# memgraph/memgraph

Hardware: AMD Instinct MI355X
Metric: edges/s PageRank (higher is better)
Workload: dtype f32; 1 GPU; RMAT-26 PageRank (327 iters); scale=26, vertices=67108864, edges=1073741824, seed=1, accumulation=f64-per-row, parallelism=single

## Files before the change

include/mgx_analytics.h:

```cpp
#ifndef MGX_ANALYTICS_H
#define MGX_ANALYTICS_H

#include <stddef.h>
#include <stdint.h>

#ifdef __cplusplus
extern "C" {
#endif

typedef int32_t mgx_status;
#define MGX_OK 0
#define MGX_ERR_NO_DEVICE 1
#define MGX_ERR_HIP 2
#define MGX_ERR_INVALID_ARGUMENT 3
#define MGX_ERR_TOO_LARGE 4
#define MGX_ERR_OUT_OF_MEMORY 5
#define MGX_ERR_NCCL 6
#define MGX_ERR_NOT_SUPPORTED 7

const char *mgx_status_string(mgx_status s);
const char *mgx_last_error(void);

int mgx_device_count(void);

typedef struct mgx_context mgx_context;
typedef struct mgx_graph mgx_graph;

mgx_status mgx_init(int device, mgx_context **out);
mgx_status mgx_destroy(mgx_context *ctx);
mgx_status mgx_sync(mgx_context *ctx);


#define MGX_BUILD_IN_CSR 1u
#define MGX_BUILD_SYM_CSR 2u
#define MGX_BUILD_WEIGHTED 4u
#define MGX_BUILD_OUT_CSR 8u
#define MGX_BUILD_NO_PERM 16u

mgx_status mgx_graph_from_coo(mgx_context *ctx, const int64_t *src, const int64_t *dst,
                              const double *weights, int64_t n_vertices, int64_t n_edges,
                              uint32_t flags, mgx_graph **out);

mgx_status mgx_graph_rmat(mgx_context *ctx, int scale, int64_t n_edges, uint64_t seed,
                          double a, double b, double c, uint32_t flags, uint64_t weight_seed,
                          mgx_graph **out);
mgx_status mgx_graph_uniform(mgx_context *ctx, int64_t n_vertices, int64_t n_edges,
                             uint64_t seed, uint32_t flags, uint64_t weight_seed,
                             mgx_graph **out);

mgx_status mgx_graph_rmat_sharded(mgx_context *ctx, int scale, int64_t n_edges, uint64_t seed,
                                  double a, double b, double c, int64_t row_begin,
                                  int64_t row_end, mgx_graph **out);

mgx_status mgx_gen_edges_to_host(mgx_context *ctx, int rmat, int scale, int64_t n_vertices,
                                 int64_t n_edges, uint64_t seed, double a, double b,
                                 double c, int64_t *out_src, int64_t *out_dst);

mgx_status mgx_graph_destroy(mgx_context *ctx, mgx_graph *g);
int64_t mgx_graph_num_vertices(const mgx_graph *g);
int64_t mgx_graph_num_edges(const mgx_graph *g);
int64_t mgx_graph_local_edges(const mgx_graph *g);
double mgx_graph_build_ms(const mgx_graph *g);
int64_t mgx_graph_in_zero_rows(const mgx_graph *g);
int64_t mgx_graph_xcd_heavy_rows(const mgx_graph *g);


typedef struct {
  int64_t iterations;
  double iter_ms;
  double sweep_ms;
  int64_t sweep_launches;
  double csr_build_ms;
  double download_ms;
} mgx_pagerank_stats;

mgx_status mgx_pagerank(mgx_context *ctx, mgx_graph *g, int64_t max_iterations,
                        double damping_factor, double stop_epsilon, double *out_rank,
                        mgx_pagerank_stats *stats);

typedef struct mgx_pagerank_run mgx_pagerank_run;
mgx_status mgx_pagerank_start(mgx_context *ctx, mgx_graph *g, double damping_factor,
                              mgx_pagerank_run **out);
mgx_status mgx_pagerank_iterate(mgx_pagerank_run *run, int64_t n_iterations);
mgx_status mgx_pagerank_iterate_eps(mgx_pagerank_run *run, int64_t max_n,
                                    double stop_epsilon, int64_t *done);
int64_t mgx_pagerank_xcd_lds_floats(const mgx_pagerank_run *run);
int mgx_pagerank_xcd_block_threads(const mgx_pagerank_run *run);
mgx_status mgx_pagerank_timing(mgx_pagerank_run *run, double *sweep_ms, int64_t *launches);
mgx_status mgx_pagerank_finish(mgx_pagerank_run *run, double *out_rank );

mgx_status mgx_wcc(mgx_context *ctx, mgx_graph *g, int64_t *out_component,
                   int64_t *n_components);

#define MGX_BFS_AUTO 0
#define MGX_BFS_TOP_DOWN 1
#define MGX_BFS_BOTTOM_UP 2
typedef struct {
  int64_t depth;
  int64_t reached;
  int64_t entries_scanned;
  int64_t top_down_levels, bottom_up_levels;
  uint64_t bottom_up_mask;
  double ms;
} mgx_bfs_stats;
mgx_status mgx_bfs(mgx_context *ctx, mgx_graph *g, int64_t source, int directed,
                   int64_t max_depth , int mode,
                   int64_t *out_hops , int64_t *out_parent ,
                   mgx_bfs_stats *stats );

typedef struct {
  int64_t bridges, trees, depth;
  int64_t nontree_entries;
  int64_t level_launches;
  double forest_ms, ms;
} mgx_bridges_stats;
mgx_status mgx_bridges(mgx_context *ctx, mgx_graph *g, int64_t *out_u, int64_t *out_v,
                       int64_t *n_bridges, mgx_bridges_stats *stats );
// ... 94 lines not shown
```

memgraph_amd/csrc/graph_build.hip:

```cpp

#include <cstring>

#include <rocprim/rocprim.hpp>

#include "../../include/mgx_graphgen.h"
#include "mgx_device.h"
#include "mgx_xcd_deal.h"

namespace {

__global__ void k_rmat(int64_t n_edges, int scale, uint64_t mixed_seed,
                       mgx_rmat_thresholds t, int32_t *src, int32_t *dst) {
  for (int64_t i = blockIdx.x * (int64_t)blockDim.x + threadIdx.x; i < n_edges;
       i += (int64_t)gridDim.x * blockDim.x) {
    uint64_t s, d;
    mgx_rmat_edge(mixed_seed, (uint64_t)i, scale, t, &s, &d);
    src[i] = (int32_t)s;
    dst[i] = (int32_t)d;
  }
}

__global__ void k_uniform(int64_t n_edges, uint64_t mixed_seed, uint64_t n_vertices,
                          int32_t *src, int32_t *dst) {
  for (int64_t i = blockIdx.x * (int64_t)blockDim.x + threadIdx.x; i < n_edges;
       i += (int64_t)gridDim.x * blockDim.x) {
    uint64_t s, d;
    mgx_uniform_edge(mixed_seed, (uint64_t)i, n_vertices, &s, &d);
    src[i] = (int32_t)s;
    dst[i] = (int32_t)d;
  }
}

__global__ void k_weights(int64_t n_edges, uint64_t mixed_seed, float *w) {
  for (int64_t i = blockIdx.x * (int64_t)blockDim.x + threadIdx.x; i < n_edges;
       i += (int64_t)gridDim.x * blockDim.x) {
    w[i] = (float)mgx_edge_weight(mixed_seed, (uint64_t)i);
  }
}

__global__ void k_hist(int64_t n_edges, const int32_t *idx, uint32_t *counts) {
  for (int64_t i = blockIdx.x * (int64_t)blockDim.x + threadIdx.x; i < n_edges;
       i += (int64_t)gridDim.x * blockDim.x)
    atomicAdd(&counts[idx[i]], 1u);
}

__global__ void k_hist2(int64_t n_edges, const int32_t *a, const int32_t *b,
                        uint32_t *counts) {
  for (int64_t i = blockIdx.x * (int64_t)blockDim.x + threadIdx.x; i < n_edges;
       i += (int64_t)gridDim.x * blockDim.x) {
    atomicAdd(&counts[a[i]], 1u);
    atomicAdd(&counts[b[i]], 1u);
  }
}

__global__ void k_hist_ranged(int64_t n_edges, const int32_t *idx, int32_t lo, int32_t hi,
                              uint32_t *counts ) {
  for (int64_t i = blockIdx.x * (int64_t)blockDim.x + threadIdx.x; i < n_edges;
       i += (int64_t)gridDim.x * blockDim.x) {
    int32_t v = idx[i];
    if (v >= lo && v < hi) atomicAdd(&counts[v - lo], 1u);
// ... 287 lines not shown
mgx_status mgx_build_bins(mgx_context *ctx, const uint32_t *row_ptr, int64_t rows,
                          mgx_bins *bins) {
  return mgx_build_bins_range(ctx, row_ptr, row_ptr + 1, rows, true,
                              bins);
}

namespace {
__global__ void k_stripe_search(int64_t rows, const uint32_t *row_ptr, const int32_t *col,
                                int32_t boundary, uint32_t *out) {
  for (int64_t r = blockIdx.x * (int64_t)blockDim.x + threadIdx.x; r < rows;
       r += (int64_t)gridDim.x * blockDim.x) {
    uint32_t lo = row_ptr[r], hi = row_ptr[r + 1];
    while (lo < hi) {
      uint32_t mid = (lo + hi) / 2;
      if (col[mid] < boundary) lo = mid + 1;
      else hi = mid;
    }
    out[r] = lo;
  }
}

__global__ void k_xcd_search(int64_t nH, const int32_t *H, const uint32_t *row_ptr,
                             const int32_t *col, int64_t V, uint32_t *out) {
  for (int64_t s = blockIdx.x * (int64_t)blockDim.x + threadIdx.x; s < nH;
       s += (int64_t)gridDim.x * blockDim.x) {
    const int32_t r = H[s];
    const uint32_t end = row_ptr[r + 1];
    uint32_t lo = row_ptr[r];
    out[s] = lo;
    for (int x = 1; x < kXcdStripes; ++x) {
      const int32_t boundary = (int32_t)mgx_xcd_stripe_off(V, x);
      uint32_t hi = end;
      while (lo < hi) {
        const uint32_t mid = lo + (hi - lo) / 2;
        if (col[mid] < boundary) lo = mid + 1;
        else hi = mid;
      }
      out[(size_t)x * nH + s] = lo;
    }
    out[(size_t)kXcdStripes * nH + s] = end;
  }
}

__global__ void k_xcd_deal(int64_t n, const int32_t *order_sorted, const uint32_t *deg_sorted,
                           int32_t *order, uint32_t *deg) {
  for (int64_t p = blockIdx.x * (int64_t)blockDim.x + threadIdx.x; p < n;
       p += (int64_t)gridDim.x * blockDim.x) {
    const int64_t id = mgx_xcd_deal(p, n);
    order[id] = order_sorted[p];
    deg[id] = deg_sorted[p];
  }
}

mgx_status build_xcd_view(mgx_context *ctx, mgx_graph *g) {
  int heavy_min = 64;
  if (const char *e = getenv("MGX_PR_XCD_HEAVY_MIN")) {
    const int v = atoi(e);
    if (v == 8 || v == 64 || v == 1024) heavy_min = v;
  }
  const int sec = heavy_min == 8 ? 1 : heavy_min == 64 ? 2 : 3;
  g->xcd_heavy_min = heavy_min;
  g->xcd_heavy_sec = sec;
  int64_t light = 0, nH = 0;
  for (int b = 0; b < 4; ++b) (b < sec ? light : nH) += g->bins_in.count[b];
  g->xcd_nH = nH;
  if (nH == 0) return MGX_OK;
  g->xcd_H = g->bins_in.rows + light;
  MGX_HIP_TRY(mgx_hip_malloc(&g->xcd_ptr, (size_t)(kXcdStripes + 1) * nH * sizeof(uint32_t)));
  hipLaunchKernelGGL(k_xcd_search, dim3(grid_for(nH)), dim3(kBlock), 0, ctx->stream, nH,
                     g->xcd_H, g->in_row_ptr, g->in_col, g->n_vertices, g->xcd_ptr);
  for (int x = 0; x < kXcdStripes; ++x) {
    MGX_TRY(mgx_build_bins_range(ctx, g->xcd_ptr + (size_t)x * nH,
                                 g->xcd_ptr + (size_t)(x + 1) * nH, nH,
                                 false, &g->xcd_bins[x]));
  }
  mgx_bin_sections secs[kXcdStripes];
  for (int x = 0; x < kXcdStripes; ++x) (void)mgx_fill_sections(g->xcd_bins[x], &secs[x]);
  MGX_HIP_TRY(mgx_hip_malloc(&g->xcd_sec, sizeof(secs)));
  MGX_HIP_TRY(hipMemcpyAsync(g->xcd_sec, secs, sizeof(secs), hipMemcpyHostToDevice,
                             ctx->stream));
  MGX_HIP_TRY(hipStreamSynchronize(ctx->stream));
  return MGX_OK;
}
}

bool mgx_xcd_wanted(int64_t n_vertices) {
  const char *stripes = getenv("MGX_PR_STRIPES");
  if (stripes && atoi(stripes) > 0) return false;
  const char *e = getenv("MGX_PR_XCD");
  if (e && *e) return atoi(e) != 0;
  return n_vertices >= (int64_t)3 << 24;
}

mgx_status mgx_build_stripes(mgx_context *ctx, mgx_graph *g) {
  const int64_t rows = g->row_end - g->row_begin;
  const int64_t V = g->n_vertices;
  if (g->xcd) {
    g->n_stripes = 1;
    return build_xcd_view(ctx, g);
  }
  int n_stripes = 1;
  const char *env = getenv("MGX_PR_STRIPES");
  if (env && atoi(env) > 0) {
    n_stripes = atoi(env);
  } else if (g->order == nullptr) {
    const int64_t contrib_bytes = V * 4;
    n_stripes = (int)((contrib_bytes + (96 << 20) - 1) / (96 << 20));
    if (n_stripes < 1) n_stripes = 1;
  } else {
    n_stripes = 1;
  }
  if (n_stripes > 16) n_stripes = 16;
  g->n_stripes = n_stripes;
  if (n_stripes == 1) return MGX_OK;
  g->stripe_width = (V + n_stripes - 1) / n_stripes;

  MGX_HIP_TRY(mgx_hip_malloc(&g->stripe_ptr, (size_t)(n_stripes + 1) * rows * sizeof(uint32_t)));
  struct CopyK {
    static __global__ void shift(int64_t rows, const uint32_t *row_ptr, uint32_t *lo,
                                 uint32_t *hi) {
      for (int64_t r = blockIdx.x * (int64_t)blockDim.x + threadIdx.x; r < rows;
           r += (int64_t)gridDim.x * blockDim.x) {
        lo[r] = row_ptr[r];
        hi[r] = row_ptr[r + 1];
      }
    }
  };
  hipLaunchKernelGGL(CopyK::shift, dim3(grid_for(rows)), dim3(kBlock), 0, ctx->stream, rows,
                     g->in_row_ptr, g->stripe_ptr, g->stripe_ptr + (size_t)n_stripes * rows);
  for (int sIdx = 1; sIdx < n_stripes; ++sIdx) {
    hipLaunchKernelGGL(k_stripe_search, dim3(grid_for(rows)), dim3(kBlock), 0, ctx->stream,
                       rows, g->in_row_ptr, g->in_col,
                       (int32_t)((int64_t)sIdx * g->stripe_width),
                       g->stripe_ptr + (size_t)sIdx * rows);
  }
// ... 261 lines not shown
```

memgraph_amd/csrc/mgx_api.cpp:

```cpp

#include <atomic>
#include <cstdarg>
#include <cstdio>
#include <cstring>

#include "mgx_internal.h"

namespace {
thread_local char g_error[1024] = {0};
}

void mgx_set_error(const char *fmt, ...) {
  va_list ap;
  va_start(ap, fmt);
  vsnprintf(g_error, sizeof(g_error), fmt, ap);
  va_end(ap);
}

extern "C" const char *mgx_last_error(void) { return g_error; }

extern "C" const char *mgx_status_string(mgx_status s) {
  switch (s) {
    case MGX_OK: return "ok";
    case MGX_ERR_NO_DEVICE: return "no HIP device";
// ... 328 lines not shown
  if (row_begin < 0 || row_end < row_begin) {
    mgx_set_error("bad shard range [%lld,%lld)", (long long)row_begin, (long long)row_end);
    return MGX_ERR_INVALID_ARGUMENT;
  }
  MGX_HIP_TRY(hipSetDevice(ctx->device));
  mgx_graph *g = nullptr;
  mgx_status s;
  {
    mgx_scope coo(ctx);
    int32_t *d_src = nullptr, *d_dst = nullptr;
    MGX_TRY(coo.alloc_plain(&d_src, n_edges));
    MGX_TRY(coo.alloc_plain(&d_dst, n_edges));
    s = mgx_gen_rmat_device(ctx, scale, n_edges, seed, a, b, c, d_src, d_dst);
    if (s == MGX_OK) {
      g = new mgx_graph();
      const int64_t clamped_end = row_end < V ? row_end : V;
      s = mgx_build_sharded_in_csr(ctx, d_src, d_dst, V, n_edges, row_begin, clamped_end, g);
      if (s == MGX_OK) {
        g->row_end = row_end;
      }
    }
  }
  if (s != MGX_OK) {
    if (g) (void)mgx_graph_destroy(ctx, g);
    return s;
  }
  *out = g;
  return MGX_OK;
}

extern "C" mgx_status mgx_graph_destroy(mgx_context *ctx, mgx_graph *g) {
  if (!g) return MGX_OK;
  (void)ctx;
  if (g->in_row_ptr) (void)hipFree(g->in_row_ptr);
  if (g->in_col) (void)hipFree(g->in_col);
  if (g->out_degree) (void)hipFree(g->out_degree);
  if (g->inv_outdeg) (void)hipFree(g->inv_outdeg);
  if (g->out_row_ptr) (void)hipFree(g->out_row_ptr);
  if (g->out_col) (void)hipFree(g->out_col);
  if (g->in_w) (void)hipFree(g->in_w);
  if (g->bins_out.rows) (void)hipFree(g->bins_out.rows);
  if (g->sym_row_ptr) (void)hipFree(g->sym_row_ptr);
  if (g->sym_col) (void)hipFree(g->sym_col);
  if (g->sym_w) (void)hipFree(g->sym_w);
  if (g->bins_in.rows) (void)hipFree(g->bins_in.rows);
  if (g->bins_sym.rows) (void)hipFree(g->bins_sym.rows);
  if (g->stripe_ptr) (void)hipFree(g->stripe_ptr);
  if (g->order) (void)hipFree(g->order);
  for (int i = 0; i < 16; ++i) {
    if (g->stripe_bins[i].rows) (void)hipFree(g->stripe_bins[i].rows);
  }
  if (g->xcd_ptr) (void)hipFree(g->xcd_ptr);
  if (g->xcd_sec) (void)hipFree(g->xcd_sec);
  for (int i = 0; i < 8; ++i) {
    if (g->xcd_bins[i].rows) (void)hipFree(g->xcd_bins[i].rows);
  }
  if (!g->uniq_alias) {
    if (g->uniq_row_ptr) (void)hipFree(g->uniq_row_ptr);
    if (g->uniq_col) (void)hipFree(g->uniq_col);
  }
  if (g->uniq_bins.rows) (void)hipFree(g->uniq_bins.rows);
  delete g;
  return MGX_OK;
}

extern "C" int64_t mgx_graph_num_vertices(const mgx_graph *g) { return g->n_vertices; }
extern "C" int64_t mgx_graph_num_edges(const mgx_graph *g) { return g->n_edges; }
extern "C" int64_t mgx_graph_local_edges(const mgx_graph *g) { return g->in_edges; }
extern "C" double mgx_graph_build_ms(const mgx_graph *g) { return g->build_ms; }
extern "C" int64_t mgx_graph_in_zero_rows(const mgx_graph *g) { return g->bins_in.n_zero; }
extern "C" int64_t mgx_graph_xcd_heavy_rows(const mgx_graph *g) {
  return g->xcd ? g->xcd_nH : -1;
}

extern "C" mgx_status mgx_wcc(mgx_context *ctx, mgx_graph *g, int64_t *out_component,
                              int64_t *n_components) {
  MGX_HIP_TRY(hipSetDevice(ctx->device));
  return mgx_wcc_impl(ctx, g, out_component, n_components);
}

extern "C" mgx_status mgx_bfs(mgx_context *ctx, mgx_graph *g, int64_t source, int directed,
                              int64_t max_depth, int mode, int64_t *out_hops,
                              int64_t *out_parent, mgx_bfs_stats *stats) {
  MGX_HIP_TRY(hipSetDevice(ctx->device));
  return mgx_bfs_impl(ctx, g, source, directed, max_depth, mode, out_hops, out_parent, stats);
}

extern "C" mgx_status mgx_bridges(mgx_context *ctx, mgx_graph *g, int64_t *out_u,
                                  int64_t *out_v, int64_t *n_bridges,
                                  mgx_bridges_stats *stats) {
  MGX_HIP_TRY(hipSetDevice(ctx->device));
  return mgx_bridges_impl(ctx, g, out_u, out_v, n_bridges, stats);
}

extern "C" mgx_status mgx_bridges_state(mgx_context *ctx, mgx_graph *g, int64_t *parent,
                                        int64_t *level, int64_t *pre, int64_t *nd,
                                        int64_t *low, int64_t *high) {
  MGX_HIP_TRY(hipSetDevice(ctx->device));
  return mgx_bridges_state_impl(ctx, g, parent, level, pre, nd, low, high);
}

extern "C" void mgx_bridges_last_stage_ms(double *forest, double *sorts_scans, double *sweep,
                                          double *levels) {
  mgx_bridges_last_stage_ms_impl(forest, sorts_scans, sweep, levels);
}

extern "C" mgx_status mgx_similarity_pairs(mgx_context *ctx, mgx_graph *g, int metric,
                                           int mode, const int64_t *u, const int64_t *v,
                                           int64_t n_pairs, double *out_sim,
                                           int64_t *out_common, mgx_similarity_stats *stats) {
  MGX_HIP_TRY(hipSetDevice(ctx->device));
  return mgx_similarity_pairs_impl(ctx, g, metric, mode, u, v, n_pairs, out_sim, out_common,
                                   stats);
}

extern "C" mgx_status mgx_similarity_all(mgx_context *ctx, mgx_graph *g, int metric,
                                         double *out_sim, mgx_similarity_stats *stats) {
  MGX_HIP_TRY(hipSetDevice(ctx->device));
  return mgx_similarity_all_impl(ctx, g, metric, out_sim, stats);
}

extern "C" mgx_status mgx_katz(mgx_context *ctx, mgx_graph *g, double alpha, double epsilon,
                               double *out_centrality, int64_t *iterations) {
  MGX_HIP_TRY(hipSetDevice(ctx->device));
  return mgx_katz_impl(ctx, g, alpha, epsilon, out_centrality, iterations);
}
// ... 13 lines not shown
```

memgraph_amd/csrc/mgx_internal.h:

```cpp
#ifndef MGX_INTERNAL_H
#define MGX_INTERNAL_H

#include <hip/hip_runtime.h>

#include <cstdint>
#include <cstdio>
#include <map>
#include <mutex>
#include <string>
#include <unordered_map>
#include <vector>

#include "../../include/mgx_analytics.h"

void mgx_set_error(const char *fmt, ...);

#define MGX_HIP_TRY(expr)                                                     \
  do {                                                                        \
    hipError_t _e = (expr);                                                   \
    if (_e != hipSuccess) {                                                   \
      mgx_set_error("%s:%d: %s failed: %s", __FILE__, __LINE__, #expr,        \
                    hipGetErrorString(_e));                                   \
      (void)hipGetLastError();  \
      return MGX_ERR_HIP;                                                     \
// ... 74 lines not shown
  int64_t count[4] = {0, 0, 0, 0};
  int64_t n_zero = 0;
  int64_t grid[4] = {0, 0, 0, 0};
  int64_t total_grid() const { return grid[0] + grid[1] + grid[2] + grid[3]; }
};

inline int64_t mgx_bin_grid(int b, int64_t count) {
  const int64_t rows_per_block[4] = {64, 16, 4, 1};
  const int64_t cap[4] = {2048, 2048, 2048, 8192};
  const int64_t need = (count + rows_per_block[b] - 1) / rows_per_block[b];
  return count ? (need < cap[b] ? need : cap[b]) : 0;
}

struct mgx_graph {
  int64_t n_vertices = 0;
  int64_t n_edges = 0;
  uint32_t flags = 0;

  uint32_t *in_row_ptr = nullptr;
  int32_t *in_col = nullptr;
  int64_t in_edges = 0;
  int64_t row_begin = 0, row_end = 0;

  uint32_t *out_degree = nullptr;
  float *inv_outdeg = nullptr;
  int32_t *order = nullptr;

  uint32_t *out_row_ptr = nullptr;
  int32_t *out_col = nullptr;

  float *in_w = nullptr;

  uint32_t *sym_row_ptr = nullptr;
  int32_t *sym_col = nullptr;
  float *sym_w = nullptr;

  mgx_bins bins_in;
  mgx_bins bins_sym;
  mgx_bins bins_out;

  int n_stripes = 1;
  int64_t stripe_width = 0;
  uint32_t *stripe_ptr = nullptr;
  mgx_bins stripe_bins[16];

  bool xcd = false;
  int xcd_heavy_min = 0;
  int xcd_heavy_sec = 4;
  int64_t xcd_nH = 0;
  const int32_t *xcd_H = nullptr;
  uint32_t *xcd_ptr = nullptr;
  mgx_bins xcd_bins[8];
  struct mgx_bin_sections *xcd_sec = nullptr;

  uint32_t *uniq_row_ptr = nullptr;
  int32_t *uniq_col = nullptr;
  int64_t uniq_entries = 0;
  bool uniq_alias = false;
  mgx_bins uniq_bins;
  bool uniq_bins_built = false;

  double build_ms = 0.0;
};

mgx_status mgx_build_from_device_coo(mgx_context *ctx, const int32_t *d_src,
                                     const int32_t *d_dst, const float *d_w,
                                     int64_t n_vertices, int64_t n_edges, uint32_t flags,
                                     mgx_graph *g);
mgx_status mgx_gen_rmat_device(mgx_context *ctx, int scale, int64_t n_edges, uint64_t seed,
                               double a, double b, double c, int32_t *d_src, int32_t *d_dst);
mgx_status mgx_gen_uniform_device(mgx_context *ctx, int64_t n_vertices, int64_t n_edges,
                                  uint64_t seed, int32_t *d_src, int32_t *d_dst);
mgx_status mgx_gen_weights_device(mgx_context *ctx, int64_t n_edges, uint64_t seed, float *d_w);
mgx_status mgx_build_bins(mgx_context *ctx, const uint32_t *row_ptr, int64_t rows,
                          mgx_bins *bins);
mgx_status mgx_build_bins_range(mgx_context *ctx, const uint32_t *lo, const uint32_t *hi,
                                int64_t rows, bool include_zero, mgx_bins *bins);
mgx_status mgx_build_bins_range(mgx_scope &own, const uint32_t *lo, const uint32_t *hi,
                                int64_t rows, bool include_zero, mgx_bins *bins);
mgx_status mgx_build_stripes(mgx_context *ctx, mgx_graph *g);
bool mgx_xcd_wanted(int64_t n_vertices);

mgx_status mgx_build_sharded_in_csr(mgx_context *ctx, const int32_t *d_src,
                                    const int32_t *d_dst, int64_t n_vertices,
                                    int64_t n_edges, int64_t row_begin, int64_t row_end,
                                    mgx_graph *g);

struct mgx_pagerank_run {
  mgx_context *ctx = nullptr;
  mgx_graph *g = nullptr;
  double damping = 0.85;
  float *rank[2] = {nullptr, nullptr};
  float *contrib[2] = {nullptr, nullptr};
  int cur = 0;
  uint32_t *d_delta = nullptr;
  double *d_scratch = nullptr;
  double *d_partial = nullptr;
  int xcd_grid = 0;
  int xcd_block = 0;
  int64_t xcd_lds_floats = 0;
  bool skip_zero = true;
  int64_t iterations = 0;
  std::vector<hipEvent_t> ev_start, ev_stop;
  int64_t ev_used = 0;
  double sweep_ms_acc = 0.0;
  int64_t launches_acc = 0;
// ... 49 lines not shown
```

memgraph_amd/csrc/pagerank.hip:

```cpp

#include <chrono>

#include "mgx_device.h"
#include "mgx_xcd_deal.h"

namespace {

struct PrArgs {
  const uint32_t *row_ptr;
  const int32_t *col;
  mgx_bin_sections bins;
  const float *contrib_old;
  const float *rank_old;
  float *rank_new;
  float *contrib_new;
  const float *inv_outdeg;
  int64_t row_base;
  float base_term;
  float damping;
  uint32_t *delta_max;
  const uint32_t *sp_lo;
  const uint32_t *sp_hi;
  double *partial;
  int mode;
// ... 70 lines not shown
}

__device__ inline void pr_finish_row(const PrArgs &A, int32_t row, double acc, float &maxd) {
  const float newr = (float)((double)A.base_term + (double)A.damping * acc);
  const int64_t gv = A.row_base + row;
  A.rank_new[gv] = newr;
  A.contrib_new[gv] = newr * A.inv_outdeg[gv];
  if (A.delta_max) {
    const float d = fabsf(newr - A.rank_old[gv]);
    if (d > maxd) maxd = d;
  }
}

__device__ inline void pr_fold_delta(const PrArgs &A, float maxd) {
  block_reduce_atomic(
      maxd, 0.0f, [](float a, float b) { return fmaxf(a, b); },
      [&](float m) { atomicMax(A.delta_max, __float_as_uint(m)); });
}

template <int LANES>
__device__ inline float pr_rows(const PrArgs &A, int sec, int64_t block_in_sec) {
  float maxd = 0.0f;
  reduce_bin_rows<LANES>(
      A.bins, sec, block_in_sec, 0.0, mgx_op_add(),
      [&](int32_t row, int sub) {
        return pr_row_sum<LANES>(A, row, sub, PrLoadGlobal{A.contrib_old});
      },
      [&](int32_t row, double acc) {
        if (A.mode == 1) {
          A.partial[row] = acc;
        } else if (A.mode == 2) {
          A.partial[row] += acc;
        } else {
          if (A.mode == 3) acc += A.partial[row];
          pr_finish_row(A, row, acc, maxd);
        }
      });
  return maxd;
}

__global__ void __launch_bounds__(kBlock) k_pr_sweep(PrArgs A) {
  float maxd = 0.0f;
  for_bin_section(A.bins.goff, [&](auto lanes, int sec, int64_t bis) {
    maxd = pr_rows<decltype(lanes)::value>(A, sec, bis);
  });
  if (A.delta_max) pr_fold_delta(A, maxd);
}

struct PrXcdArgs {
  const int32_t *col;
  const float *contrib_old;
  double *partial;
  const mgx_bin_sections *sec;
  const uint32_t *xptr;
  int64_t nH;
  int64_t V;
  uint32_t hot_k;
};

template <bool HOT, int THREADS>
__global__ void __launch_bounds__(THREADS) k_pr_sweep_xcd(PrXcdArgs X) {
  const int x = blockIdx.x % kXcdStripes;
  const mgx_bin_sections &S = X.sec[x];
  PrArgs A;
  A.col = X.col;
  A.sp_lo = X.xptr + (size_t)x * X.nH;
  A.sp_hi = A.sp_lo + X.nH;
  double *out = X.partial + (size_t)x * X.nH;
  const int64_t block = blockIdx.x / kXcdStripes;
  const int64_t nblocks = gridDim.x / kXcdStripes;
  auto sweep = [&](auto load) {
    auto section = [&](auto lanes, int sec) {
      constexpr int L = decltype(lanes)::value;
      reduce_rows<L, THREADS>(
          S.rows + S.off[sec], S.n[sec], block, nblocks, 0.0, mgx_op_add(),
          [&](int32_t slot, int sub) { return pr_row_sum<L>(A, slot, sub, load); },
          [&](int32_t slot, double acc) { out[slot] = acc; });
    };
    section(std::integral_constant<int, 256>{}, 3);
    section(std::integral_constant<int, 64>{}, 2);
    section(std::integral_constant<int, 16>{}, 1);
    section(std::integral_constant<int, 4>{}, 0);
  };
  if constexpr (HOT) {
    extern __shared__ float hot[];
    const int64_t base = mgx_xcd_stripe_off(X.V, x);
    const int64_t len = mgx_xcd_stripe_off(X.V, x + 1) - base;
    const uint32_t kx = len < (int64_t)X.hot_k ? (uint32_t)len : X.hot_k;
    for (uint32_t i = threadIdx.x; i < kx; i += THREADS) hot[i] = X.contrib_old[base + i];
    __syncthreads();
    sweep(PrLoadHot{X.contrib_old, hot, (uint32_t)base, kx});
  } else {
    sweep(PrLoadGlobal{X.contrib_old});
  }
}

using pr_xcd_kernel = void (*)(PrXcdArgs);
constexpr int kXcdDefaultWidth = 1024;

pr_xcd_kernel pr_xcd_kernel_for(bool hot, int threads) {
  switch (threads) {
    case 256: return hot ? k_pr_sweep_xcd<true, 256> : k_pr_sweep_xcd<false, 256>;
    case 1024: return hot ? k_pr_sweep_xcd<true, 1024> : k_pr_sweep_xcd<false, 1024>;
    default: return nullptr;
  }
}

__global__ void __launch_bounds__(kBlock)
k_pr_finish_heavy(PrArgs A, const int32_t *H, const uint32_t *xptr, int64_t nH) {
  float maxd = 0.0f;
  for (int64_t s = blockIdx.x * (int64_t)blockDim.x + threadIdx.x; s < nH;
       s += (int64_t)gridDim.x * blockDim.x) {
    double acc = 0.0;
    uint32_t lo = xptr[s];
    for (int x = 0; x < kXcdStripes; ++x) {
      const uint32_t hi = xptr[(size_t)(x + 1) * nH + s];
      if (hi > lo) acc += A.partial[(size_t)x * nH + s];
      lo = hi;
    }
    pr_finish_row(A, H[s], acc, maxd);
  }
  if (A.delta_max) pr_fold_delta(A, maxd);
}

__global__ void k_pr_init(int64_t n, float r0, const float *inv, float *rank,
                          float *contrib) {
  for (int64_t i = blockIdx.x * (int64_t)blockDim.x + threadIdx.x; i < n;
       i += (int64_t)gridDim.x * blockDim.x) {
    rank[i] = r0;
    contrib[i] = r0 * inv[i];
  }
}

__global__ void k_sum_f32(int64_t n, const float *x, double *out) {
  double acc = 0.0;
  for (int64_t i = blockIdx.x * (int64_t)blockDim.x + threadIdx.x; i < n;
       i += (int64_t)gridDim.x * blockDim.x)
    acc += (double)x[i];
  block_reduce_atomic(acc, 0.0, mgx_op_add(), [&](double s) { atomicAdd(out, s); });
}

__global__ void k_pr_widen(int64_t n, const float *rank, const double *sum,
                           const int32_t *order, double *out) {
  const double inv = 1.0 / *sum;
  for (int64_t i = blockIdx.x * (int64_t)blockDim.x + threadIdx.x; i < n;
       i += (int64_t)gridDim.x * blockDim.x)
    out[order ? order[i] : i] = (double)rank[i] * inv;
}

int64_t pr_fill_sections(const mgx_pagerank_run *run, const mgx_bins &bins,
                         mgx_bin_sections *s) {
  const int64_t nz = bins.n_zero;
  if (!run->skip_zero || run->dist || run->iterations < 2 || nz == 0)
    return mgx_fill_sections(bins, s);
  mgx_bins rest = bins;
  rest.count[0] -= nz;
  rest.grid[0] = mgx_bin_grid(0, rest.count[0]);
  const int64_t goff = mgx_fill_sections(rest, s);
  for (int b = 0; b < 4; ++b) s->off[b] += nz;
  return goff;
}

mgx_status queue_xcd_sweep(mgx_pagerank_run *run, PrArgs A) {
  mgx_context *ctx = run->ctx;
  mgx_graph *g = run->g;
  const int64_t nH = g->xcd_nH;
  if (nH > 0) {
    PrXcdArgs X;
    X.col = g->in_col;
    X.contrib_old = A.contrib_old;
    X.partial = run->d_partial;
    X.sec = g->xcd_sec;
    X.xptr = g->xcd_ptr;
    X.nH = nH;
    X.V = g->n_vertices;
    X.hot_k = (uint32_t)run->xcd_lds_floats;
    hipLaunchKernelGGL(pr_xcd_kernel_for(X.hot_k > 0, run->xcd_block),
                       dim3((uint32_t)run->xcd_grid), dim3((uint32_t)run->xcd_block),
                       (size_t)X.hot_k * sizeof(float), ctx->stream, X);
  }
  mgx_bins light = g->bins_in;
  for (int b = g->xcd_heavy_sec; b < 4; ++b) light.count[b] = light.grid[b] = 0;
  const int64_t goff = pr_fill_sections(run, light, &A.bins);
  A.sp_lo = g->in_row_ptr;
  A.sp_hi = g->in_row_ptr + 1;
  A.mode = 0;
  if (goff > 0) {
    hipLaunchKernelGGL(k_pr_sweep, dim3((uint32_t)goff), dim3(kBlock), 0, ctx->stream, A);
  }
  if (nH > 0) {
    hipLaunchKernelGGL(k_pr_finish_heavy, dim3((uint32_t)grid_for(nH)), dim3(kBlock), 0,
                       ctx->stream, A, g->xcd_H, (const uint32_t *)g->xcd_ptr, nH);
  }
  return MGX_OK;
}

mgx_status queue_one_iteration(mgx_pagerank_run *run, bool track_delta) {
  mgx_context *ctx = run->ctx;
  mgx_graph *g = run->g;
  const int64_t V = g->n_vertices;

  PrArgs A;
  A.row_ptr = g->in_row_ptr;
  A.col = g->in_col;
  A.contrib_old = run->contrib[run->cur];
  A.rank_old = run->rank[run->cur];
  A.rank_new = run->rank[1 - run->cur];
  A.contrib_new = run->contrib[1 - run->cur];
  A.inv_outdeg = g->inv_outdeg;
  A.row_base = g->row_begin;
  A.base_term = (float)((1.0 - run->damping) / (double)V);
  A.damping = (float)run->damping;
  A.delta_max = track_delta ? run->d_delta : nullptr;
  A.partial = run->d_partial;

  if (track_delta) MGX_HIP_TRY(hipMemsetAsync(run->d_delta, 0, 4, ctx->stream));

  const int n_stripes = g->n_stripes;
  const int64_t rows = (g->row_end < V ? g->row_end : V) - g->row_begin;
  if (V > 0) {
    if (run->ev_used >= (int64_t)run->ev_start.size()) {
      hipEvent_t e0, e1;
      MGX_HIP_TRY(hipEventCreate(&e0));
      MGX_HIP_TRY(hipEventCreate(&e1));
      run->ev_start.push_back(e0);
      run->ev_stop.push_back(e1);
// ... 354 lines not shown
```

memgraph_amd/native.py:

```python
import ctypes
import os

import numpy as np

_DIR = os.path.dirname(os.path.abspath(__file__))
LIB_PATH = os.path.join(_DIR, "lib", "libmgx_analytics.so")

BUILD_IN_CSR = 1
BUILD_SYM_CSR = 2
BUILD_WEIGHTED = 4
BUILD_OUT_CSR = 8
BUILD_NO_PERM = 16

UNIQUE_ID_BYTES = 128

_I64 = ctypes.POINTER(ctypes.c_int64)
_F64 = ctypes.POINTER(ctypes.c_double)


class PagerankStats(ctypes.Structure):
    _fields_ = [
        ("iterations", ctypes.c_int64),
        ("iter_ms", ctypes.c_double),
        ("sweep_ms", ctypes.c_double),
# ... 22 lines not shown

class BridgesStats(ctypes.Structure):
    _fields_ = [
        ("bridges", ctypes.c_int64),
        ("trees", ctypes.c_int64),
        ("depth", ctypes.c_int64),
        ("nontree_entries", ctypes.c_int64),
        ("level_launches", ctypes.c_int64),
        ("forest_ms", ctypes.c_double),
        ("ms", ctypes.c_double),
    ]


SIM_JACCARD = 0
SIM_OVERLAP = 1
SIM_AUTO = 0
SIM_SEARCH = 1
SIM_MERGE = 2


class SimilarityStats(ctypes.Structure):
    _fields_ = [
        ("pairs", ctypes.c_int64),
        ("search_pairs", ctypes.c_int64),
        ("merge_pairs", ctypes.c_int64),
        ("distinct_entries", ctypes.c_int64),
        ("chunks", ctypes.c_int64),
        ("prep_ms", ctypes.c_double),
        ("ms", ctypes.c_double),
    ]


ERR_OUT_OF_MEMORY = 5


class MgxError(RuntimeError):
    def __init__(self, message, status=None):
        super().__init__(message)
        self.status = status


class Native:
    def __init__(self, path=LIB_PATH):
        if not os.path.exists(path):
            raise MgxError(f"{path} not built — run `make` / __graft_entry__.build()")
        self.lib = ctypes.CDLL(path)
        self.lib.mgx_status_string.restype = ctypes.c_char_p
        self.lib.mgx_last_error.restype = ctypes.c_char_p
        self.lib.mgx_graph_build_ms.restype = ctypes.c_double
        self.lib.mgx_graph_num_vertices.restype = ctypes.c_int64
        self.lib.mgx_graph_num_edges.restype = ctypes.c_int64
        self.lib.mgx_graph_local_edges.restype = ctypes.c_int64
        self.lib.mgx_graph_xcd_heavy_rows.restype = ctypes.c_int64
        self.lib.mgx_graph_in_zero_rows.restype = ctypes.c_int64
        self.lib.mgx_pagerank_xcd_lds_floats.restype = ctypes.c_int64

    def _check(self, status, what):
        if status != 0:
            msg = self.lib.mgx_status_string(status).decode()
            detail = self.lib.mgx_last_error().decode()
            raise MgxError(f"{what}: {msg} ({detail})", status)

    def device_count(self):
        return self.lib.mgx_device_count()

    def init(self, device=0):
        ctx = ctypes.c_void_p()
        self._check(self.lib.mgx_init(device, ctypes.byref(ctx)), "mgx_init")
        return ctx

    def destroy(self, ctx):
        self.lib.mgx_destroy(ctx)

    def sync(self, ctx):
        self._check(self.lib.mgx_sync(ctx), "mgx_sync")

    def test_scope_hook(self, fail_at=-1):
        self.lib.mgx_test_scope_hook.restype = ctypes.c_int64
        return self.lib.mgx_test_scope_hook(ctypes.c_int64(fail_at))

    def graph_from_coo(self, ctx, src, dst, n_vertices, weights=None, flags=BUILD_IN_CSR):
        src = np.ascontiguousarray(src, dtype=np.int64)
        dst = np.ascontiguousarray(dst, dtype=np.int64)
        pw = None
        if weights is not None:
            weights = np.ascontiguousarray(weights, dtype=np.float64)
            pw = weights.ctypes.data_as(_F64)
        g = ctypes.c_void_p()
        self._check(
            self.lib.mgx_graph_from_coo(ctx, src.ctypes.data_as(_I64),
                                        dst.ctypes.data_as(_I64), pw,
                                        ctypes.c_int64(n_vertices),
                                        ctypes.c_int64(len(src)), ctypes.c_uint32(flags),
                                        ctypes.byref(g)), "mgx_graph_from_coo")
        return g

    def graph_rmat(self, ctx, scale, n_edges, seed=1, a=0.57, b=0.19, c=0.19,
                   flags=BUILD_IN_CSR, weight_seed=7):
        g = ctypes.c_void_p()
        self._check(
            self.lib.mgx_graph_rmat(ctx, ctypes.c_int(scale), ctypes.c_int64(n_edges),
                                    ctypes.c_uint64(seed), ctypes.c_double(a),
                                    ctypes.c_double(b), ctypes.c_double(c),
                                    ctypes.c_uint32(flags), ctypes.c_uint64(weight_seed),
                                    ctypes.byref(g)), "mgx_graph_rmat")
        return g

    def graph_uniform(self, ctx, n_vertices, n_edges, seed=42, flags=BUILD_IN_CSR,
                      weight_seed=7):
        g = ctypes.c_void_p()
        self._check(
            self.lib.mgx_graph_uniform(ctx, ctypes.c_int64(n_vertices),
                                       ctypes.c_int64(n_edges), ctypes.c_uint64(seed),
                                       ctypes.c_uint32(flags), ctypes.c_uint64(weight_seed),
                                       ctypes.byref(g)), "mgx_graph_uniform")
        return g

    def graph_rmat_sharded(self, ctx, scale, n_edges, row_begin, row_end, seed=1, a=0.57,
                           b=0.19, c=0.19):
        g = ctypes.c_void_p()
        self._check(
            self.lib.mgx_graph_rmat_sharded(ctx, ctypes.c_int(scale),
                                            ctypes.c_int64(n_edges), ctypes.c_uint64(seed),
                                            ctypes.c_double(a), ctypes.c_double(b),
                                            ctypes.c_double(c), ctypes.c_int64(row_begin),
                                            ctypes.c_int64(row_end), ctypes.byref(g)),
            "mgx_graph_rmat_sharded")
        return g

    def graph_destroy(self, ctx, g):
        self.lib.mgx_graph_destroy(ctx, g)

    def graph_build_ms(self, g):
        return self.lib.mgx_graph_build_ms(g)

    def graph_xcd_heavy_rows(self, g):
        return self.lib.mgx_graph_xcd_heavy_rows(g)

    def graph_in_zero_rows(self, g):
        return self.lib.mgx_graph_in_zero_rows(g)

    def pagerank(self, ctx, g, n_vertices, max_iterations=100, damping=0.85, eps=1e-5):
        out = np.zeros(n_vertices, dtype=np.float64)
        stats = PagerankStats()
        self._check(
            self.lib.mgx_pagerank(ctx, g, ctypes.c_int64(max_iterations),
                                  ctypes.c_double(damping), ctypes.c_double(eps),
                                  out.ctypes.data_as(_F64), ctypes.byref(stats)),
            "mgx_pagerank")
        return out, stats

    def pagerank_start(self, ctx, g, damping=0.85):
        run = ctypes.c_void_p()
        self._check(self.lib.mgx_pagerank_start(ctx, g, ctypes.c_double(damping),
                                                ctypes.byref(run)), "mgx_pagerank_start")
        return run

    def pagerank_start_dist(self, ctx, g, row_begin, row_end, damping=0.85):
        run = ctypes.c_void_p()
        self._check(
            self.lib.mgx_pagerank_start_dist(ctx, g, ctypes.c_double(damping),
                                             ctypes.c_int64(row_begin),
                                             ctypes.c_int64(row_end), ctypes.byref(run)),
            "mgx_pagerank_start_dist")
        return run

    def pagerank_iterate(self, run, n):
        self._check(self.lib.mgx_pagerank_iterate(run, ctypes.c_int64(n)),
                    "mgx_pagerank_iterate")

    def pagerank_xcd_lds_floats(self, run):
        return self.lib.mgx_pagerank_xcd_lds_floats(run)

    def pagerank_xcd_block_threads(self, run):
        return self.lib.mgx_pagerank_xcd_block_threads(run)

    def pagerank_timing(self, run):
        ms = ctypes.c_double()
        n = ctypes.c_int64()
        self._check(self.lib.mgx_pagerank_timing(run, ctypes.byref(ms), ctypes.byref(n)),
                    "mgx_pagerank_timing")
        return ms.value, n.value

    def pagerank_finish(self, run, n_vertices=0, want_rank=True):
        out = np.zeros(n_vertices, dtype=np.float64) if want_rank else None
        p = out.ctypes.data_as(_F64) if want_rank and n_vertices else None
        self._check(self.lib.mgx_pagerank_finish(run, p), "mgx_pagerank_finish")
        return out

    def wcc(self, ctx, g, n_vertices):
# ... 287 lines not shown
```

Measured before the change: 170.3 billion edges/s.

## Repack XCD stripe column segments into contiguous per-stripe aligned column streams

At graph build time, copies each heavy row's per-XCD-stripe column segment into a new column array grouped by stripe, so that every stripe's segments sit contiguously. Segments of rows in the two heaviest bins are padded to 4-int alignment that matches their source offset. The PageRank XCD kernel then reads these new lo/hi pointers and the packed column array instead of the interleaved CSR. The goal is to cut the cache lines touched per stripe sweep and improve streaming locality, at the cost of extra device memory for a second column copy and more build-time work.

```diff
diff --git a/experiments/stream_lines.py b/experiments/stream_lines.py
--- /dev/null
+++ b/experiments/stream_lines.py
@@ -0,0 +1,72 @@
+import os
+import sys
+
+import numpy as np
+
+sys.path.insert(0, os.path.dirname(os.path.dirname(os.path.abspath(__file__))))
+from memgraph_amd.rmat import gen_rmat
+
+STRIPES, GRANULE, ALIGN = 8, 16, 32
+
+
+def stripe_off(nv, x):
+    g = (nv + GRANULE - 1) // GRANULE
+    rem = g % STRIPES
+    off = ((g // STRIPES) * x + min(rem, x)) * GRANULE
+    if g and (g - 1) % STRIPES < x:
+        off -= g * GRANULE - nv
+    return off
+
+
+def segments(scale):
+    nv = 1 << scale
+    src, dst = gen_rmat(scale, 16 << scale, seed=1)
+    hot = np.argsort(-np.bincount(src, minlength=nv), kind="stable")
+    p = np.arange(nv)
+    q = p // GRANULE
+    off = np.array([stripe_off(nv, x) for x in range(STRIPES + 1)])
+    new_id = np.empty(nv, dtype=np.int64)
+    new_id[hot] = off[q % STRIPES] + (q // STRIPES) * GRANULE + p % GRANULE
+    nsrc, ndst = new_id[src], new_id[dst]
+    indeg = np.bincount(ndst, minlength=nv)
+    row_ptr = np.concatenate([[0], np.cumsum(indeg)])
+    stripe_of = np.searchsorted(off, nsrc, side="right") - 1
+    length = np.bincount(ndst * STRIPES + stripe_of, minlength=nv * STRIPES).reshape(nv, STRIPES)
+    start = row_ptr[:-1, None] + np.cumsum(length, axis=1) - length
+    return start, length, indeg
+
+
+def lines(start, length, line_bytes):
+    per = line_bytes // 4
+    return int(((start + length - 1) // per - start // per + 1).sum())
+
+
+def stream_ints(start, length):
+    total = 0
+    for x in range(STRIPES):
+        lo, ln = start[:, x], length[:, x]
+        wide = ln >= 64
+        ints = int(((((lo[wide] & 3) + ln[wide] + 3) >> 2) << 2).sum()) + int(ln[~wide].sum())
+        total += (ints + ALIGN - 1) // ALIGN * ALIGN
+    return total
+
+
+def main():
+    scales = [int(a) for a in sys.argv[1:]] or [20, 22]
+    print("scale rows share_of_E segments mean median x64 x128 stream_ints/ints")
+    for scale in scales:
+        start, length, indeg = segments(scale)
+        edges = int(indeg.sum())
+        for name, rows in (("in-degree>=64", indeg >= 64), ("in-degree8..63", (indeg >= 8) & (indeg < 64))):
+            s, ln = start[rows].ravel(), length[rows].ravel()
+            keep = ln > 0
+            s, ln = s[keep], ln[keep]
+            ints = int(ln.sum())
+            ratios = [lines(s, ln, b) / -(-ints * 4 // b) for b in (64, 128)]
+            stream = stream_ints(start[rows], length[rows]) / ints
+            print(f"{scale} {name} {ints / edges:.2f} {len(ln):.2e} {ln.mean():.1f} "
+                  f"{int(np.median(ln))} x{ratios[0]:.2f} x{ratios[1]:.2f} {stream:.4f}")
+
+
+if __name__ == "__main__":
+    main()
diff --git a/include/mgx_analytics.h b/include/mgx_analytics.h
--- a/include/mgx_analytics.h
+++ b/include/mgx_analytics.h
@@ -63,6 +63,7 @@
 double mgx_graph_build_ms(const mgx_graph *g);
 int64_t mgx_graph_in_zero_rows(const mgx_graph *g);
 int64_t mgx_graph_xcd_heavy_rows(const mgx_graph *g);
+int64_t mgx_graph_xcd_stream_ints(const mgx_graph *g);
 
 
 typedef struct {
diff --git a/memgraph_amd/csrc/graph_build.hip b/memgraph_amd/csrc/graph_build.hip
--- a/memgraph_amd/csrc/graph_build.hip
+++ b/memgraph_amd/csrc/graph_build.hip
@@ -6,6 +6,7 @@
 #include "../../include/mgx_graphgen.h"
 #include "mgx_device.h"
 #include "mgx_xcd_deal.h"
+#include "mgx_xcd_stream.h"
 
 namespace {
 
@@ -399,6 +400,142 @@
   }
 }
 
+struct xcd_stream_lists {
+  const int32_t *rows[kXcdStripes * 4];
+  int64_t n[kXcdStripes * 4];
+  int64_t first[kXcdStripes * 4 + 1];
+  uint32_t base[kXcdStripes];
+};
+
+__global__ void k_xcd_stream_allot(xcd_stream_lists L, const uint32_t *xptr, int64_t nH,
+                                   uint32_t *allot) {
+  for (int k = 0; k < kXcdStripes * 4; ++k) {
+    const int x = k / 4, sec = 3 - k % 4;
+    for (int64_t i = blockIdx.x * (int64_t)blockDim.x + threadIdx.x; i < L.n[k];
+         i += (int64_t)gridDim.x * blockDim.x) {
+      const int32_t slot = L.rows[k][i];
+      const uint32_t lo = xptr[(size_t)x * nH + slot];
+      const uint32_t hi = xptr[(size_t)(x + 1) * nH + slot];
+      allot[L.first[k] + i] = mgx_xcd_seg_allot(lo, hi - lo, mgx_xcd_seg_aligned(sec));
+    }
+  }
+}
+
+__global__ void __launch_bounds__(kBlock)
+k_xcd_stream_fill(xcd_stream_lists L, const uint32_t *xptr, int64_t nH, const int32_t *col,
+                  const uint32_t *rel, int32_t *scol, uint32_t *slo, uint32_t *shi) {
+  for (int x = 0; x < kXcdStripes; ++x) {
+    auto section = [&](auto lanes, int sec) {
+      constexpr int LANES = decltype(lanes)::value;
+      const int k = x * 4 + (3 - sec);
+      const bool aligned = mgx_xcd_seg_aligned(sec);
+      for_row_steps<LANES>(
+          L.rows[k], L.n[k], blockIdx.x, gridDim.x, [&](const int32_t *rowp, bool live, int sub) {
+            if (!live) return;
+            const int32_t slot = *rowp;
+            const int64_t item = L.first[k] + (rowp - L.rows[k]);
+            const uint32_t lo = xptr[(size_t)x * nH + slot];
+            const uint32_t len = xptr[(size_t)(x + 1) * nH + slot] - lo;
+            const uint32_t pos = L.base[x] + rel[item];
+            const uint32_t start = mgx_xcd_seg_start(pos, lo, aligned);
+            for (uint32_t j = sub; j < len; j += LANES) scol[start + j] = col[lo + j];
+            if (sub == 0) {
+              slo[(size_t)x * nH + slot] = start;
+              shi[(size_t)x * nH + slot] = start + len;
+              const uint32_t end = pos + mgx_xcd_seg_allot(lo, len, aligned);
+              for (uint32_t j = pos; j < start; ++j) scol[j] = 0;
+              for (uint32_t j = start + len; j < end; ++j) scol[j] = 0;
+            }
+          });
+    };
+    section(std::integral_constant<int, 256>{}, 3);
+    section(std::integral_constant<int, 64>{}, 2);
+    section(std::integral_constant<int, 16>{}, 1);
+    section(std::integral_constant<int, 4>{}, 0);
+  }
+}
+
+mgx_status build_xcd_stream(mgx_context *ctx, mgx_graph *g) {
+  if (const char *e = getenv("MGX_PR_XCD_STREAM")) {
+    if (*e && atoi(e) == 0) return MGX_OK;
+  }
+  const int64_t nH = g->xcd_nH;
+  xcd_stream_lists L = {};
+  int64_t items = 0, aligned_items = 0;
+  for (int x = 0; x < kXcdStripes; ++x) {
+    mgx_bin_sections S;
+    (void)mgx_fill_sections(g->xcd_bins[x], &S);
+    for (int sec = 3; sec >= 0; --sec) {
+      const int k = x * 4 + (3 - sec);
+      L.rows[k] = S.rows + S.off[sec];
+      L.n[k] = S.n[sec];
+      L.first[k] = items;
+      items += S.n[sec];
+      if (mgx_xcd_seg_aligned(sec)) aligned_items += S.n[sec];
+    }
+  }
+  L.first[kXcdStripes * 4] = items;
+  if (items == 0) return MGX_OK;
+  const uint64_t most = (uint64_t)g->in_edges + 6ull * (uint64_t)aligned_items +
+                        (uint64_t)kXcdStripes * kXcdStreamAlign;
+  if (most > 0xFFFFFFFFull) return MGX_OK;
+
+  mgx_scope bufs(ctx);
+  uint32_t *allot = nullptr, *rel = nullptr;
+  MGX_TRY(bufs.alloc(&allot, items));
+  MGX_TRY(bufs.alloc(&rel, items));
+  hipLaunchKernelGGL(k_xcd_stream_allot, dim3(grid_for(items)), dim3(kBlock), 0, ctx->stream, L,
+                     (const uint32_t *)g->xcd_ptr, nH, allot);
+  uint32_t last_rel[kXcdStripes] = {0}, last_allot[kXcdStripes] = {0};
+  for (int x = 0; x < kXcdStripes; ++x) {
+    const int64_t first = L.first[x * 4], n = L.first[x * 4 + 4] - first;
+    if (n == 0) continue;
+    MGX_TRY(mgx_with_temp(ctx, "column stream scan", [&](void *tmp, size_t &bytes) {
+      return rocprim::exclusive_scan(tmp, bytes, allot + first, rel + first, 0u, n,
+                                     rocprim::plus<uint32_t>(), ctx->stream);
+    }));
+    MGX_HIP_TRY(hipMemcpyAsync(&last_rel[x], rel + first + n - 1, 4, hipMemcpyDeviceToHost,
+                               ctx->stream));
+    MGX_HIP_TRY(hipMemcpyAsync(&last_allot[x], allot + first + n - 1, 4, hipMemcpyDeviceToHost,
+                               ctx->stream));
+  }
+  MGX_HIP_TRY(hipStreamSynchronize(ctx->stream));
+  uint64_t end[kXcdStripes], total = 0;
+  for (int x = 0; x < kXcdStripes; ++x) {
+    L.base[x] = (uint32_t)total;
+    end[x] = total + last_rel[x] + last_allot[x];
+    total = mgx_xcd_stream_round(end[x]);
+  }
+  if (total > most) {
+    mgx_set_error("column stream: %llu ints exceed the bound %llu",
+                  (unsigned long long)total, (unsigned long long)most);
+    return MGX_ERR_TOO_LARGE;
+  }
+
+  MGX_HIP_TRY(mgx_hip_malloc(&g->xcd_scol, (size_t)total * sizeof(int32_t)));
+  MGX_HIP_TRY(mgx_hip_malloc(&g->xcd_slo, (size_t)kXcdStripes * nH * sizeof(uint32_t)));
+  MGX_HIP_TRY(mgx_hip_malloc(&g->xcd_shi, (size_t)kXcdStripes * nH * sizeof(uint32_t)));
+  MGX_HIP_TRY(hipMemsetAsync(g->xcd_slo, 0, (size_t)kXcdStripes * nH * sizeof(uint32_t),
+                             ctx->stream));
+  MGX_HIP_TRY(hipMemsetAsync(g->xcd_shi, 0, (size_t)kXcdStripes * nH * sizeof(uint32_t),
+                             ctx->stream));
+  for (int x = 0; x < kXcdStripes; ++x) {
+    const uint64_t next = mgx_xcd_stream_round(end[x]);
+    if (next > end[x]) {
+      MGX_HIP_TRY(hipMemsetAsync(g->xcd_scol + end[x], 0, (size_t)(next - end[x]) * sizeof(int32_t),
+                                 ctx->stream));
+    }
+  }
+  hipLaunchKernelGGL(k_xcd_stream_fill, dim3(grid_for(items, 8192)), dim3(kBlock), 0,
+                     ctx->stream, L, (const uint32_t *)g->xcd_ptr, nH,
+                     (const int32_t *)g->in_col, (const uint32_t *)rel, g->xcd_scol, g->xcd_slo,
+                     g->xcd_shi);
+  MGX_HIP_TRY(hipGetLastError());
+  MGX_HIP_TRY(hipStreamSynchronize(ctx->stream));
+  g->xcd_stream_ints = (int64_t)total;
+  return MGX_OK;
+}
+
 mgx_status build_xcd_view(mgx_context *ctx, mgx_graph *g) {
   int heavy_min = 64;
   if (const char *e = getenv("MGX_PR_XCD_HEAVY_MIN")) {
@@ -427,7 +564,7 @@
   MGX_HIP_TRY(hipMemcpyAsync(g->xcd_sec, secs, sizeof(secs), hipMemcpyHostToDevice,
                              ctx->stream));
   MGX_HIP_TRY(hipStreamSynchronize(ctx->stream));
-  return MGX_OK;
+  return build_xcd_stream(ctx, g);
 }
 }
 
diff --git a/memgraph_amd/csrc/mgx_api.cpp b/memgraph_amd/csrc/mgx_api.cpp
--- a/memgraph_amd/csrc/mgx_api.cpp
+++ b/memgraph_amd/csrc/mgx_api.cpp
@@ -404,6 +404,9 @@
   }
   if (g->xcd_ptr) (void)hipFree(g->xcd_ptr);
   if (g->xcd_sec) (void)hipFree(g->xcd_sec);
+  if (g->xcd_scol) (void)hipFree(g->xcd_scol);
+  if (g->xcd_slo) (void)hipFree(g->xcd_slo);
+  if (g->xcd_shi) (void)hipFree(g->xcd_shi);
   for (int i = 0; i < 8; ++i) {
     if (g->xcd_bins[i].rows) (void)hipFree(g->xcd_bins[i].rows);
   }
@@ -424,6 +427,9 @@
 extern "C" int64_t mgx_graph_xcd_heavy_rows(const mgx_graph *g) {
   return g->xcd ? g->xcd_nH : -1;
 }
+extern "C" int64_t mgx_graph_xcd_stream_ints(const mgx_graph *g) {
+  return g->xcd_scol ? g->xcd_stream_ints : -1;
+}
 
 extern "C" mgx_status mgx_wcc(mgx_context *ctx, mgx_graph *g, int64_t *out_component,
                               int64_t *n_components) {
diff --git a/memgraph_amd/csrc/mgx_internal.h b/memgraph_amd/csrc/mgx_internal.h
--- a/memgraph_amd/csrc/mgx_internal.h
+++ b/memgraph_amd/csrc/mgx_internal.h
@@ -150,6 +150,10 @@
   uint32_t *xcd_ptr = nullptr;
   mgx_bins xcd_bins[8];
   struct mgx_bin_sections *xcd_sec = nullptr;
+  int32_t *xcd_scol = nullptr;
+  uint32_t *xcd_slo = nullptr;
+  uint32_t *xcd_shi = nullptr;
+  int64_t xcd_stream_ints = -1;
 
   uint32_t *uniq_row_ptr = nullptr;
   int32_t *uniq_col = nullptr;
diff --git a/memgraph_amd/csrc/mgx_xcd_stream.h b/memgraph_amd/csrc/mgx_xcd_stream.h
--- /dev/null
+++ b/memgraph_amd/csrc/mgx_xcd_stream.h
@@ -0,0 +1,22 @@
+#ifndef MGX_XCD_STREAM_H
+#define MGX_XCD_STREAM_H
+
+#include "mgx_xcd_deal.h"
+
+constexpr uint32_t kXcdStreamAlign = 32;
+
+MGX_HD inline bool mgx_xcd_seg_aligned(int sec) { return sec >= 2; }
+
+MGX_HD inline uint32_t mgx_xcd_seg_allot(uint32_t lo, uint32_t len, bool aligned) {
+  return aligned ? ((lo & 3u) + len + 3u) & ~3u : len;
+}
+
+MGX_HD inline uint32_t mgx_xcd_seg_start(uint32_t pos, uint32_t lo, bool aligned) {
+  return aligned ? pos + (lo & 3u) : pos;
+}
+
+MGX_HD inline uint64_t mgx_xcd_stream_round(uint64_t end) {
+  return (end + kXcdStreamAlign - 1) / kXcdStreamAlign * kXcdStreamAlign;
+}
+
+#endif
diff --git a/memgraph_amd/csrc/pagerank.hip b/memgraph_amd/csrc/pagerank.hip
--- a/memgraph_amd/csrc/pagerank.hip
+++ b/memgraph_amd/csrc/pagerank.hip
@@ -146,7 +146,7 @@
   const float *contrib_old;
   double *partial;
   const mgx_bin_sections *sec;
-  const uint32_t *xptr;
+  const uint32_t *lo, *hi;
   int64_t nH;
   int64_t V;
   uint32_t hot_k;
@@ -158,8 +158,8 @@
   const mgx_bin_sections &S = X.sec[x];
   PrArgs A;
   A.col = X.col;
-  A.sp_lo = X.xptr + (size_t)x * X.nH;
-  A.sp_hi = A.sp_lo + X.nH;
+  A.sp_lo = X.lo + (size_t)x * X.nH;
+  A.sp_hi = X.hi + (size_t)x * X.nH;
   double *out = X.partial + (size_t)x * X.nH;
   const int64_t block = blockIdx.x / kXcdStripes;
   const int64_t nblocks = gridDim.x / kXcdStripes;
@@ -261,11 +261,18 @@
   const int64_t nH = g->xcd_nH;
   if (nH > 0) {
     PrXcdArgs X;
-    X.col = g->in_col;
+    if (g->xcd_scol) {
+      X.col = g->xcd_scol;
+      X.lo = g->xcd_slo;
+      X.hi = g->xcd_shi;
+    } else {
+      X.col = g->in_col;
+      X.lo = g->xcd_ptr;
+      X.hi = g->xcd_ptr + nH;
+    }
     X.contrib_old = A.contrib_old;
     X.partial = run->d_partial;
     X.sec = g->xcd_sec;
-    X.xptr = g->xcd_ptr;
     X.nH = nH;
     X.V = g->n_vertices;
     X.hot_k = (uint32_t)run->xcd_lds_floats;
diff --git a/memgraph_amd/native.py b/memgraph_amd/native.py
--- a/memgraph_amd/native.py
+++ b/memgraph_amd/native.py
@@ -98,6 +98,7 @@
         self.lib.mgx_graph_num_edges.restype = ctypes.c_int64
         self.lib.mgx_graph_local_edges.restype = ctypes.c_int64
         self.lib.mgx_graph_xcd_heavy_rows.restype = ctypes.c_int64
+        self.lib.mgx_graph_xcd_stream_ints.restype = ctypes.c_int64
         self.lib.mgx_graph_in_zero_rows.restype = ctypes.c_int64
         self.lib.mgx_pagerank_xcd_lds_floats.restype = ctypes.c_int64
 
@@ -182,6 +183,9 @@
 
     def graph_xcd_heavy_rows(self, g):
         return self.lib.mgx_graph_xcd_heavy_rows(g)
+
+    def graph_xcd_stream_ints(self, g):
+        return self.lib.mgx_graph_xcd_stream_ints(g)
 
     def graph_in_zero_rows(self, g):
         return self.lib.mgx_graph_in_zero_rows(g)
```

Measured after the change: 172.9 billion edges/s, median of 6. 1.02x the previous value.
